# innate2adaptive/decombinator

Measured on AMD Instinct MI355X. Metric: Mreads/s decombined (150 bp human-beta), higher is better.
Workload: dtype u8

## Files before the change

### decombinator_amd/csrc/dcrx_kernels_v2.hip

```cpp
#include <hip/hip_runtime.h>
#include <hip/hip_ext.h>

#include <algorithm>
#include <cstddef>
#include <cstdio>
#include <cstdlib>
#include <vector>

#include "../../include/dcrx.h"
#include "dcrx_device.h"
#include "dcrx_launch.h"
#include "dcrx_dcr_device.h"
#include "dcrx_v2_device.h"
#include "dcrx_sink_device.h"

namespace dcrx {

bool first_use_on_device(bool (&seen)[64]);
void attributes_set_on_device(bool (&seen)[64]);

constexpr int DCRX_V2_BLOCK = 1024;
#ifdef DCRX_SCAN_STAMPS
__device__ uint32_t *g_scan_stamps;
#endif
// ... 287 lines not shown
  if (tid < DCRX_N_COUNTERS) lds_counts[tid] = 0;
  if (tid < V2_WK_WORDS) lds_work[tid] = 0;
  {
    const uint4 *src = reinterpret_cast<const uint4 *>(V0.trans);
    uint4 *dst = reinterpret_cast<uint4 *>(lds_trans);
    for (uint32_t i = tid; i < V0.trans_bytes / 16; i += blockDim.x) dst[i] = src[i];
  }
  const V2Tab tab{};
  uint32_t *lds_side = lds_work + V2_WK_WORDS;
  uint32_t *lds_bk = lds_side + (T0.lds_image_bytes - T0.dfa_bytes) / 4;
  uint32_t *ring = lds_bk + V0.bk_bytes / 4;
  const uint32_t ring_mask = 64u * ring_batches - 1u;
  constexpr uint32_t ES = (uint32_t)v2_ering_stride<NW>(), ering_mask = 64u * V2_ERING_BATCHES - 1u;
  uint32_t *ring2 = ring + (size_t)(ring_mask + 1u) * V2_RING_STRIDE;
  uint32_t *lds_dry = ring2 + (size_t)(ering_mask + 1u) * ES;
  if (FUSE >= 0) {
    {
      const uint4 *s1 = reinterpret_cast<const uint4 *>(T0.image + T0.dfa_bytes), *s2 = reinterpret_cast<const uint4 *>(V0.bk);
      uint4 *d1 = reinterpret_cast<uint4 *>(lds_side), *d2 = reinterpret_cast<uint4 *>(lds_bk);
      for (uint32_t i = tid; i < (T0.lds_image_bytes - T0.dfa_bytes) / 16; i += blockDim.x) d1[i] = s1[i];
      for (uint32_t i = tid; i < V0.bk_bytes / 16; i += blockDim.x) d2[i] = s2[i];
    }
    for (uint32_t i = tid; i <= ring_mask; i += blockDim.x) { ring[i * V2_RING_STRIDE + NW] = 0u; ring[i * V2_RING_STRIDE + NW + 1] = 0u; }
    if (FUSE_E) for (uint32_t i = tid; i <= ering_mask; i += blockDim.x) { ring2[i * ES + NW] = 0u; ring2[i * ES + NW + 1] = 0u; }
  }
  __syncthreads();
  const uint32_t nw = B.stride >> 2;
  const int lane = tid & 63;
  const unsigned long long lt_mask = (1ull << lane) - 1ull;
  const bool tagged = B.n_reads < (1ull << 30);

  const uint64_t blk_lo = (uint64_t)blockIdx.x * per_block;
  const uint64_t blk_hi = blk_lo + per_block < B.n_reads ? blk_lo + per_block : B.n_reads;
  uint32_t e_lo = 0u, e_hi = 0u;
  if (B.n_exc) {
    v2_exc_slice(B, blk_lo < blk_hi ? blk_lo : blk_hi, blk_hi, lds_work + V2_WK_EXC, tid);
    e_lo = lds_work[V2_WK_EXC]; e_hi = lds_work[V2_WK_EXC + 2];
    v2_exc_marks(B, e_lo, e_hi, true, tid);
    asm volatile("s_waitcnt vmcnt(0)" ::: "memory");
// ... 252 lines not shown
  }
  if (FUSE >= 0 && lane == 0) {
    asm volatile("s_waitcnt lgkmcnt(0)" ::: "memory");
    atomicAdd(&lds_work[V2_WK_SCANNED], 1u);
  }
  }
  if (FUSE_E && (wv >= n_scan_waves + tw || (DCRX_V2_HELP_DRAIN && scans))) {
   if constexpr (FUSE_E) {
    constexpr bool REV = FUSE == 1;
#if DCRX_V2_PRIO_TAIL
    __builtin_amdgcn_s_setprio(DCRX_V2_PRIO_TAIL);
#endif
    uint32_t kw_base[K_NCLASS];
#pragma unroll
    for (int c = 0; c < K_NCLASS; c++) kw_base[c] = T0.kw_base[c];
    const Rescue2Tabs rt = rescue2_tabs(T0, V0, reinterpret_cast<const uint8_t *>(lds_side), reinterpret_cast<const uint8_t *>(lds_bk), REV, kw_base);
    const Counters C{lds_counts}, Cdry{lds_dry};
    constexpr uint32_t nb_mask = V2_ERING_BATCHES - 1u, nb_shift = (uint32_t)__builtin_ctz(V2_ERING_BATCHES);
    constexpr uint32_t V2_RING_EXIT = 0xFFFFFFFFu;
    for (uint32_t spins = 0;;) {
      uint32_t c = 0, nvalid = 0;
      if (lane == 0) {
        c = __hip_atomic_load(&lds_work[V2_WK_CLAIM2], __ATOMIC_RELAXED, __HIP_MEMORY_SCOPE_WORKGROUP);
        const bool mine = __hip_atomic_load(&lds_work[V2_WK_GEN2 + (c & nb_mask)], __ATOMIC_RELAXED, __HIP_MEMORY_SCOPE_WORKGROUP) == (c >> nb_shift);
        const uint32_t f = __hip_atomic_load(&lds_work[V2_WK_FILLED2 + (c & nb_mask)], __ATOMIC_RELAXED, __HIP_MEMORY_SCOPE_WORKGROUP);
        if (!mine) nvalid = 0;
        else if (f == 64u) nvalid = 64u;
        else if (__hip_atomic_load(&lds_work[V2_WK_SCANNED], __ATOMIC_RELAXED, __HIP_MEMORY_SCOPE_WORKGROUP) == n_scan_waves) {
          const uint32_t h = __hip_atomic_load(&lds_work[V2_WK_HEAD2], __ATOMIC_RELAXED, __HIP_MEMORY_SCOPE_WORKGROUP);
          const uint32_t rem = h - 64u * c;
          nvalid = (int32_t)rem <= 0 ? V2_RING_EXIT : min(rem, 64u);
// ... 3 lines not shown
          if (!__hip_atomic_compare_exchange_strong(&lds_work[V2_WK_CLAIM2], &expect, c + 1u, __ATOMIC_RELAXED, __ATOMIC_RELAXED, __HIP_MEMORY_SCOPE_WORKGROUP)) nvalid = 0;
        }
      }
      c = (uint32_t)__builtin_amdgcn_readfirstlane((int)c);
      nvalid = (uint32_t)__builtin_amdgcn_readfirstlane((int)nvalid);
      if (nvalid == V2_RING_EXIT) break;
      if (!nvalid) {
        if (++spins > (1u << 24)) { if (lane == 0) atomicAdd(&counters[DCRX_C_DEVICE_ERRORS], 1ull); break; }
        __builtin_amdgcn_s_sleep(4);
        continue;
      }
      asm volatile("s_waitcnt lgkmcnt(0)" ::: "memory");
      uint32_t *sl = ring2 + ((64u * c + (uint32_t)lane) & ering_mask) * ES;
      int status = -2;
      uint32_t errs = 0, x0 = 0;
      uint32_t lg[NW];
#pragma unroll
      for (int k = 0; k < NW; k++) lg[k] = 0u;
      if ((uint32_t)lane < nvalid) {
        x0 = sl[NW + 2];
#pragma unroll
        for (int k = 0; k < NW; k++) lg[k] = sl[NW + 3 + k];
        const uint32_t dg = sl[2 * NW + 3];
        const uint32_t r = x0 & V2_R_MASK;
        const int n = UNIFORM_LEN ? (int)B.read_len : (int)B.lens[r];
        const LdsWords lw{dcrx_ldsaddr_of(sl)};
        auto on_ok = [&](dcrx_record_t rec, const uint32_t) {
          rec.frame = (uint8_t)(o ? 0 : 1);
          DCRX_STORE_FINISH(records + r, rec);
        };
        status = rescue2_fast_to<REV, NW, V2_SHAPE_ONE>(rt, lw, lg, n, cfg, on_ok, errs, *Tmem, C, Cdry, dg);
        if (status > 0) {
          dcrx_record_t rec;
          rec.v = rec.j = rec.v_start = rec.j_end = rec.ins_start = rec.ins_len = 0; rec.vdel = rec.jdel = 0;
          rec.status = (uint8_t)status; rec.frame = (uint8_t)(o ? 0 : 1);
          DCRX_STORE_FINISH(records + r, rec);
        } else if (status < 0) errs = 0;
      }
      v2_tally_rescue(lds_counts, lane, status, errs, o == 0);
      if (__builtin_expect(status == RESCUE2_SLOW, 0)) {
        uint32_t ww[NW];
#pragma unroll
        for (int k = 0; k < NW; k++) ww[k] = sl[k];
        if (!v2_left_push<NW>(Q.left, queue_count, x0, lg, ww)) v2_hand_over(B, queue, gqueue, qcap, queue_count, tagged, x0 & V2_R_MASK, false);
      }
      asm volatile("s_waitcnt lgkmcnt(0)" ::: "memory");
      if (lane == 0) {
        __hip_atomic_store(&lds_work[V2_WK_FILLED2 + (c & nb_mask)], 0u, __ATOMIC_RELAXED, __HIP_MEMORY_SCOPE_WORKGROUP);
        asm volatile("s_waitcnt lgkmcnt(0)" ::: "memory");
        atomicAdd(&lds_work[V2_WK_GEN2 + (c & nb_mask)], 1u);
      }
      spins = 0;
    }
   }
  }
  if (FUSE >= 0 && (DCRX_V2_HELP_DRAIN || (wv >= n_scan_waves && wv < n_scan_waves + tw))) {
   if constexpr (FUSE >= 0) {
    constexpr bool REV = FUSE == 1;
// ... 129 lines not shown
    x0e = (int)lo;
    while (lo < B.n_exc && B.exc_read[lo] == r) lo++;
    x1e = (int)lo;
    ExcLayout xl;
    if (x1e - x0e > V2_MAX_EXC && !exc_layout(B.exc_pos, B.exc_chr, x0e, x1e, xl)) {
      v2_hand_over(B, queue, gqueue, qcap, queue_count, tagged, r, true); return;
    }
  }
  if (!finish2_words<UNIFORM_LEN, NW, ORI>(T, V, B, cfg, (uint64_t)r, w, ev, (x0 & V2_R_JMULTI) != 0u, x0e, x1e, C, records))
    v2_hand_over(B, queue, gqueue, qcap, queue_count, tagged, r, exc);
}

constexpr int V2_LEFT_SLOTS = 15;
struct V2FinishLds {
  uint32_t *counts, *side, *bk, *strip, *dry, *left;
};
template <int NW, int BLOCK>
__device__ __forceinline__ V2FinishLds v2_finish_layout(const DevTables &T0, const V2Ori &V, uint32_t *smem, const int tid) {
  V2FinishLds L;
  L.counts = smem;
  L.side = smem + DCRX_N_COUNTERS;
  L.bk = L.side + (T0.lds_image_bytes - T0.dfa_bytes) / 4;
  L.strip = L.bk + V.bk_bytes / 4 + (uint32_t)tid * lds_words_stride<NW>();
  L.dry = L.bk + V.bk_bytes / 4 + (uint32_t)BLOCK * lds_words_stride<NW>();
  L.left = L.dry + DCRX_N_COUNTERS + (uint32_t)(tid >> 6) * (1 + V2_LEFT_SLOTS);
  return L;
}
template <int NW, int BLOCK>
__device__ __forceinline__ V2FinishLds v2_finish_stage(const DevTables &T0, const V2Ori &V, uint32_t *smem, const int tid) {
  const V2FinishLds L = v2_finish_layout<NW, BLOCK>(T0, V, smem, tid);
  if (tid < DCRX_N_COUNTERS) L.counts[tid] = 0;
  stage_lds<BLOCK>(T0.image + T0.dfa_bytes, L.side, (T0.lds_image_bytes - T0.dfa_bytes) / 16, 0, 0, tid);
  stage_lds<BLOCK>(V.bk, L.bk, V.bk_bytes / 16, 0, 0, tid);
  L.strip[NW] = 0u; L.strip[NW + 1] = 0u;
  if ((tid & 63) == 0) L.left[0] = 0u;
  return L;
}
template <int NW>
static uint32_t v2_finish_block_lds(const DevTables &T, int o, int block) {
  return DCRX_N_COUNTERS * 4 + (T.lds_image_bytes - T.dfa_bytes) + T.v2[o].bk_bytes + (uint32_t)block * lds_words_stride<NW>() * 4 + DCRX_N_COUNTERS * 4 +
         (uint32_t)(block / 64) * (1 + V2_LEFT_SLOTS) * 4;
}

__device__ __forceinline__ void v2_note_left(uint32_t *left, const uint32_t slot, const BatchDev &B, uint32_t *__restrict__ queue, uint32_t *__restrict__ gqueue,
                                             const uint32_t qcap, uint32_t *__restrict__ queue_count, const uint32_t r, const bool exc) {
  const uint32_t at = atomicAdd(&left[0], 1u);
  if (at < (uint32_t)V2_LEFT_SLOTS) left[1 + at] = slot;
  else v2_hand_over(B, queue, gqueue, qcap, queue_count, B.n_reads < (1ull << 30), r, exc);
}
template <int NW>
struct V2EntryWords { uint32_t lg[NW], w[NW]; };
template <bool UNIFORM_LEN, int NW, int ORI>
__device__ __forceinline__ void v2_tail_jobs(const Tail2Tabs &tt, const V2FinishLds &L, const BatchDev &B, const CfgDev &cfg, dcrx_record_t *__restrict__ records,
                                             const V2Lists &Q, const uint32_t n_regions, const uint32_t split, uint32_t *__restrict__ queue,
                                             uint32_t *__restrict__ gqueue, const uint32_t qcap, uint32_t *__restrict__ queue_count,
                                             const DevTables *__restrict__ Tmem, const uint32_t gwave, const uint32_t n_gwaves, const int tid, const V2SinkCall &S) {
// ... 104 lines not shown
      uint32_t x[2 + 2 * NW];
      const bool more = next_first < en;
      uint32_t after_raw = 0;
      uint32_t nf = next_first;
      if constexpr (AHEAD) {
#pragma unroll
        for (int k = 0; k < 2 + 2 * NW; k++) x[k] = x1[k];
        nf = v2_landed(x, next_first);
      }
      if (more && lane == 0) after_raw = __hip_atomic_fetch_add(tickets + V2_L_COUNTS * region + V2_L_TICKETS, which == V2_L_E ? 1u : 0x10000u, __ATOMIC_RELAXED, __HIP_MEMORY_SCOPE_AGENT);
      if constexpr (AHEAD) {
        v2_get_rows<2 + 2 * NW>(l.rows, l.cap, nf + lane, nf + lane < en, x1);
      } else {
        v2_get_rows<2 + 2 * NW>(l.rows, l.cap, first + lane, first + lane < en, x);
      }
      uint32_t lg[NW], w[NW];
#pragma unroll
      for (int k = 0; k < NW; k++) { lg[k] = x[1 + k]; w[k] = x[1 + NW + k]; }
      int status = -2;
      uint32_t errs = 0;
      uint64_t tup = 0;
      const uint32_t r = x[0] & V2_R_MASK;
      if (first + lane < en) {
        status = RESCUE2_SLOW;
        if (!(x[0] & V2_R_EXC)) {
          const int n = UNIFORM_LEN ? (int)B.read_len : (int)B.lens[r];
#pragma unroll
          for (int k = 0; k < NW; k++) strip[k] = w[k];
          auto on_ok = [&](dcrx_record_t rec, const uint32_t e) {
            rec.frame = (uint8_t)(o ? 0 : 1);
            DCRX_STORE_FINISH(records + r, rec);
            if (S.dev) tup = sink_tuple_lean(rec, S.wpack, (e & 8u) != 0u && 2 * rt.split[1] != (int)rt.t.L[1]);
          };
          if (which == V2_L_E) status = rescue2_fast_to<ORI == 1, NW, V2_SHAPE_ONE>(rt, lw, lg, n, cfg, on_ok, errs, *Tmem, C, Cdry, x[1 + 2 * NW]);
          else status = rescue2_fast_to<ORI == 1, NW, V2_SHAPE_BOTH>(rt, lw, lg, n, cfg, on_ok, errs, *Tmem, C, Cdry, x[1 + 2 * NW]);
          if (status > 0) {
            dcrx_record_t rec;
            rec.v = rec.j = rec.v_start = rec.j_end = rec.ins_start = rec.ins_len = 0; rec.vdel = rec.jdel = 0;
            rec.status = (uint8_t)status; rec.frame = (uint8_t)(o ? 0 : 1);
            DCRX_STORE_FINISH(records + r, rec);
          } else if (status < 0) errs = 0;
        }
      }
      v2_tally_rescue(lds_counts, lane, status, errs, o == 0);
      if (S.dev) sink_put(S, region, which == V2_L_E ? S.e_off : S.c_off, first + (uint32_t)lane, first + lane < en, status == DCRX_S_OK, r, tup, lane, nullptr);
      if (__builtin_expect(status == RESCUE2_SLOW, 0)) v2_note_left(s_left, first + (uint32_t)lane, B, queue, gqueue, qcap, queue_count, r, (x[0] & V2_R_EXC) != 0u);
      first = next_first;
      if (more) {
        const uint32_t t = (uint32_t)__builtin_amdgcn_readfirstlane((int)after_raw);
        next_first = 64u * (split + (which == V2_L_E ? (t & 0xFFFFu) : (t >> 16)));
// ... 68 lines not shown
  A.S.items = v2_global(A.S.items); A.S.hits = v2_global(A.S.hits);
  return A;
}
template <bool UNIFORM_LEN, int NW, int ORI, bool SINK>
DCRX_V2_ROLE void v2_rescue_role(const uint32_t vblock_, const uint32_t ka_lo, const uint32_t ka_hi) {
  extern __shared__ __align__(64) uint32_t smem[];
  V2FinishLocals A = v2_finish_args(ka_lo, ka_hi);
  if constexpr (!SINK) A.S.dev = nullptr;
  const uint32_t vblock = (uint32_t)__builtin_amdgcn_readfirstlane((int)vblock_);
  const int tid = threadIdx.x;
  const V2Ori V = A.T0.v2[ORI];
  const V2FinishLds L = v2_finish_layout<NW, DCRX_V2_FBLOCK>(A.T0, V, smem, tid);
  uint32_t kw_base[K_NCLASS];
#pragma unroll
  for (int c = 0; c < K_NCLASS; c++) kw_base[c] = A.T0.kw_base[c];
  const Rescue2Tabs rt = rescue2_tabs(A.T0, V, reinterpret_cast<const uint8_t *>(L.side), reinterpret_cast<const uint8_t *>(L.bk), ORI == 1, kw_base);
  constexpr uint32_t WPB = DCRX_V2_FBLOCK / 64;
  v2_rescue_jobs<UNIFORM_LEN, NW, ORI>(rt, L, A.B, A.cfg, A.records, A.Q, A.n_regions, A.R.rsplit, A.queue, A.gqueue, A.qcap, A.queue_count, A.Tmem,
                                       vblock * WPB + (uint32_t)(tid >> 6), A.R.rgrid * WPB, tid, A.S, A.tickets);
}
template <bool UNIFORM_LEN, int NW, int ORI, bool SINK>
DCRX_V2_ROLE void v2_tail_role(const uint32_t vblock_, const uint32_t ka_lo, const uint32_t ka_hi) {
  extern __shared__ __align__(64) uint32_t smem[];
  V2FinishLocals A = v2_finish_args(ka_lo, ka_hi);
  if constexpr (!SINK) A.S.dev = nullptr;
  const uint32_t vblock = (uint32_t)__builtin_amdgcn_readfirstlane((int)vblock_);
  const int tid = threadIdx.x;
  const V2Ori V = A.T0.v2[ORI];
  const V2FinishLds L = v2_finish_layout<NW, DCRX_V2_FBLOCK>(A.T0, V, smem, tid);
  const Tail2Tabs tt = tail2_tabs(A.T0, V, reinterpret_cast<const uint8_t *>(L.side), reinterpret_cast<const uint8_t *>(L.bk), ORI == 1);
  constexpr uint32_t WPB = DCRX_V2_FBLOCK / 64;
// ... 81 lines not shown
  bool work = true;
  if (b < R.xgrid) {
    role = 0;
    const uint32_t g = b / R.bsplit;
    work = g < A.n_regions && R.width * (DCRX_V2_FBLOCK / 64) * (b % R.bsplit) < A.Q.counts[V2_L_COUNTS * g + V2_L_X];
  } else {
    b -= R.xgrid;
    const uint32_t paired = 2u * min(R.rgrid, R.tgrid);
    if (b < paired) { role = (b & 1u) ? 2 : 1; b >>= 1; }
    else { b -= paired; role = R.rgrid > R.tgrid ? 1 : 2; b += min(R.rgrid, R.tgrid); }
  }
  const V2Ori V = A.T0.v2[ORI];
  V2FinishLds L = v2_finish_layout<NW, DCRX_V2_FBLOCK>(A.T0, V, smem, tid);
  const bool staged = work || blockIdx.x == 0;
  if (staged) {
    L = v2_finish_stage<NW, DCRX_V2_FBLOCK>(A.T0, V, smem, tid);
    __syncthreads();
    if (role == 1) v2_rescue_role<UNIFORM_LEN, NW, ORI, SINK>(b, (uint32_t)ka, (uint32_t)(ka >> 32));
    else if (TAIL_ROLE && role == 2) v2_tail_role<UNIFORM_LEN, NW, ORI, SINK>(b, (uint32_t)ka, (uint32_t)(ka >> 32));
    else v2_general_role<UNIFORM_LEN, NW, ORI, SINK>(blockIdx.x == 0 ? 3u : 1u, b, (uint32_t)ka, (uint32_t)(ka >> 32));
  }
  __syncthreads();
  if (blockIdx.x != 0 && tid == 0) atomicAdd(A.queue_count + V2_QC_DONE, 1u);
  __syncthreads();
  if (staged && tid < DCRX_N_COUNTERS && L.counts[tid]) atomicAdd(&A.counters[tid], (unsigned long long)L.counts[tid]);
}

template <bool UNIFORM_LEN, int NW, int ORI>
__global__ __launch_bounds__(DCRX_V2_FBLOCK, DCRX_V2_RWAVES) void left2_kernel(const V2FinishArgs A) {
  extern __shared__ __align__(64) uint32_t smem[];
  const int tid = threadIdx.x;
  if (A.queue_count[V2_QC_LEFT] == 0u) return;
  if (tid == 0) A.queue_count[V2_QC_DONE] = A.R.xgrid + A.R.rgrid + A.R.tgrid;
  __syncthreads();
  const uint64_t ka = (uint64_t)__builtin_amdgcn_kernarg_segment_ptr();
  const V2Ori V = A.T0.v2[ORI];
  const V2FinishLds L = v2_finish_stage<NW, DCRX_V2_FBLOCK>(A.T0, V, smem, tid);
  __syncthreads();
  v2_general_role<UNIFORM_LEN, NW, ORI, false>(2u, 0u, (uint32_t)ka, (uint32_t)(ka >> 32));
  __syncthreads();
  if (tid < DCRX_N_COUNTERS && L.counts[tid]) atomicAdd(&A.counters[tid], (unsigned long long)L.counts[tid]);
}

template <bool UNIFORM_LEN, int NW, int ORI>
__global__ __launch_bounds__(DCRX_V2_TBLOCK, DCRX_V2_TWAVES) void tail2_kernel(
    DevTables T0, BatchDev B, CfgDev cfg, dcrx_record_t *__restrict__ records, unsigned long long *__restrict__ counters,
    V2Lists Q, uint32_t n_regions, uint32_t split, uint32_t *__restrict__ queue, uint32_t *__restrict__ gqueue, uint32_t qcap,
    uint32_t *__restrict__ queue_count, const DevTables *__restrict__ Tmem) {
  extern __shared__ __align__(64) uint32_t smem[];
  const int tid = threadIdx.x;
  const V2Ori V = T0.v2[ORI];
  const V2FinishLds L = v2_finish_stage<NW, DCRX_V2_TBLOCK>(T0, V, smem, tid);
  const Tail2Tabs tt = tail2_tabs(T0, V, reinterpret_cast<const uint8_t *>(L.side), reinterpret_cast<const uint8_t *>(L.bk), ORI == 1);
  __syncthreads();
  v2_tail_jobs<UNIFORM_LEN, NW, ORI>(tt, L, B, cfg, records, Q, n_regions, split, queue, gqueue, qcap, queue_count, Tmem,
                                     blockIdx.x * (DCRX_V2_TBLOCK / 64) + (uint32_t)(tid >> 6), gridDim.x * (DCRX_V2_TBLOCK / 64), tid, V2SinkCall{});
  __syncthreads();
  if (tid < DCRX_N_COUNTERS && L.counts[tid]) atomicAdd(&counters[tid], (unsigned long long)L.counts[tid]);
}

template <bool UNIFORM_LEN, int NW, int ORI>
__global__ __launch_bounds__(DCRX_V2_FBLOCK, DCRX_V2_RWAVES) void rescue2_kernel(
    DevTables T0, BatchDev B, CfgDev cfg, dcrx_record_t *__restrict__ records, unsigned long long *__restrict__ counters,
    V2Lists Q, uint32_t n_regions, uint32_t split, uint32_t *__restrict__ queue, uint32_t *__restrict__ gqueue, uint32_t qcap,
    uint32_t *__restrict__ queue_count, const DevTables *__restrict__ Tmem) {
  extern __shared__ __align__(64) uint32_t smem[];
  const int tid = threadIdx.x;
  const V2Ori V = T0.v2[ORI];
  const V2FinishLds L = v2_finish_stage<NW, DCRX_V2_FBLOCK>(T0, V, smem, tid);
  uint32_t kw_base[K_NCLASS];
#pragma unroll
  for (int c = 0; c < K_NCLASS; c++) kw_base[c] = T0.kw_base[c];
  const Rescue2Tabs rt = rescue2_tabs(T0, V, reinterpret_cast<const uint8_t *>(L.side), reinterpret_cast<const uint8_t *>(L.bk), ORI == 1, kw_base);
  __syncthreads();
  v2_rescue_jobs<UNIFORM_LEN, NW, ORI>(rt, L, B, cfg, records, Q, n_regions, split, queue, gqueue, qcap, queue_count, Tmem,
                                       blockIdx.x * (DCRX_V2_FBLOCK / 64) + (uint32_t)(tid >> 6), gridDim.x * (DCRX_V2_FBLOCK / 64), tid, V2SinkCall{}, Q.counts);
  __syncthreads();
  if (tid < DCRX_N_COUNTERS && L.counts[tid]) atomicAdd(&counters[tid], (unsigned long long)L.counts[tid]);
}

template <bool UNIFORM_LEN, int NW, int ORI>
__global__ __launch_bounds__(DCRX_V2_FBLOCK, 4) void events2_kernel(
    DevTables T0, BatchDev B, CfgDev cfg, dcrx_record_t *__restrict__ records, unsigned long long *__restrict__ counters,
    V2Lists Q, int which, uint32_t group, uint32_t width, uint32_t bsplit, uint32_t ext, uint32_t n_regions, uint32_t *__restrict__ queue, uint32_t *__restrict__ gqueue, uint32_t qcap,
    uint32_t *__restrict__ queue_count) {
  extern __shared__ __align__(64) uint32_t smem[];
  V2Ori V = T0.v2[ORI];
  const uint32_t lcap = v2_list<NW>(Q, which, 0).cap;
// ... 242 lines not shown
        if (ready) {
          float ms[2] = {0.f, 0.f};
          for (int a = 0; a < 2 * NP && ok; a++) { float t = 0.f; ok = hipEventElapsedTime(&t, eslot->ev_e[a][0], eslot->ev_e[a][1]) == hipSuccess; ms[a < NP ? 0 : 1] += t; }
          eslot->us_e[0] = 1e3f * ms[0] / NP; eslot->us_e[1] = 1e3f * ms[1] / NP;
          eslot->fuse_e = (ok && ms[1] > 0.f && ms[1] < 0.985f * ms[0]) ? 1 : 0;
          want = eslot->fuse_e == 1;
          static const bool say = dcrx_debug_env("DCRX_DEBUG_TUNE") != nullptr;
          if (say) fprintf(stderr, "dcrx tune: scan + finishing launch of %llu reads, frame %d: %.1f us with list E a role, %.1f inside the scan -> %s\n",
                           (unsigned long long)B.n_reads, o, eslot->us_e[0], eslot->us_e[1], eslot->fuse_e ? "inside the scan" : "a role");
        }
      }
      (void)hipGetLastError();
    }
    if (ring_batches && want && !retry && !(cfg.flags & ~(DCRX_F_V2_SHAPE(3)))) {
      const uint32_t fixed = v2_scan_lds_bytes(T, o) + (T.lds_image_bytes - T.dfa_bytes) + T.v2[o].bk_bytes + 64u * V2_ERING_BATCHES * (uint32_t)v2_ering_stride<NW>() * 4u +
                             DCRX_N_COUNTERS * 4u;
      for (uint32_t nb = ring_batches; nb >= 8u; nb >>= 1)
        if (fixed + nb * 64u * V2_RING_STRIDE * 4u <= 160u * 1024u) { ring_batches_e = nb; scan_lds_e = fixed + nb * 64u * V2_RING_STRIDE * 4u; break; }
      if (!ring_batches_e && eslot && fuse_e_env < 0) eslot->fuse_e = 0;
      if (ring_batches_e) {
        fuse_e = true;
        ks_e = o ? scan2_kernel<UNIFORM, NW, RPL, NARROW, PREFETCH, 1, false, true> : scan2_kernel<UNIFORM, NW, RPL, NARROW, PREFETCH, 0, false, true>;
      }
    }
  }
  if (P.tune && ring_batches) P.tune[o].last_form = 3u;
  const uint32_t scan_lds = v2_scan_lds_bytes(T, o) + (ring_batches ? (T.lds_image_bytes - T.dfa_bytes) + T.v2[o].bk_bytes + ring_batches * 64u * V2_RING_STRIDE * 4u : 0u);
  auto ke = o ? events2_kernel<UNIFORM, NW, 1> : events2_kernel<UNIFORM, NW, 0>;
  auto kt = o ? tail2_kernel<UNIFORM, NW, 1> : tail2_kernel<UNIFORM, NW, 0>;
  auto kr = o ? rescue2_kernel<UNIFORM, NW, 1> : rescue2_kernel<UNIFORM, NW, 0>;
  auto kf = o ? finish2_kernel<UNIFORM, NW, 1> : finish2_kernel<UNIFORM, NW, 0>;
// ... 357 lines not shown
```

### decombinator_amd/csrc/dcrx_v2_device.h

```cpp
#pragma once

#include "dcrx_dcr_device.h"

namespace dcrx {

#ifndef DCRX_HOST_EMUL
DCRX_DEV uint32_t dcrx_alignbit(uint32_t hi, uint32_t lo, uint32_t sh) { return __builtin_amdgcn_alignbit(hi, lo, sh); }
typedef __attribute__((address_space(3))) uint16_t dcrx_lds_u16;
struct V2Tab {};
DCRX_DEV uint32_t v2_entry(const V2Tab &, uint32_t byte_off) {
  return *reinterpret_cast<const dcrx_lds_u16 *>(static_cast<uintptr_t>(byte_off));
}
#else
inline uint32_t dcrx_alignbit(uint32_t hi, uint32_t lo, uint32_t sh) { return (uint32_t)((((uint64_t)hi << 32) | lo) >> (sh & 31)); }
struct V2Tab { const uint16_t *base; };
inline uint32_t v2_entry(const V2Tab &tab, uint32_t byte_off) { return tab.base[byte_off >> 1]; }
#endif

#ifndef DCRX_HOST_EMUL
typedef uint32_t dcrx_ldsaddr;
template <typename T>
DCRX_DEV T dcrx_lds_at(dcrx_ldsaddr a, uint32_t i) {
  return reinterpret_cast<const __attribute__((address_space(3))) T *>(static_cast<uintptr_t>(a))[i];
}
// ... 818 lines not shown
  else if (status == DCRX_S_J_WALK_FAIL) C.add(DCRX_C_VJ_ASSIGNMENT_FAILED);
  else if (status == DCRX_S_F_TOOLONG) C.add(DCRX_C_DCRFILTER_TOOLONG_INTERTAG);
  else if (status == DCRX_S_F_IMPOSS_DEL) C.add(DCRX_C_DCRFILTER_IMPOSS_DELETION);
  else if (status == DCRX_S_F_OVERLAP) C.add(DCRX_C_DCRFILTER_TAG_OVERLAP);
}

struct Rescue2Tabs {
  Tail2Tabs t;
  uint32_t h_mask[2][2];
  dcrx_ldsaddr h_kw[2][2], h_pk[2][2];
  dcrx_ldsaddr kw_begin, kw_tags;
  dcrx_ldsaddr tag_pk[2];
  uint32_t kw_base[2][2];
  uint32_t Lh[2][2];
  int32_t split[2];
};

DCRX_DEV Rescue2Tabs rescue2_tabs(const DevTables &T0, const V2Ori &V0, const uint8_t *side, const uint8_t *bk, const bool rev,
                                  const uint32_t (&kw_base)[K_NCLASS]) {
  Rescue2Tabs r;
  r.t = tail2_tabs(T0, V0, side, bk, rev);
  auto at_side = [&](const void *p) { return dcrx_ldsaddr_of(side + ((reinterpret_cast<const uint8_t *>(p) - T0.image) - T0.dfa_bytes)); };
  for (int g = 0; g < 2; g++) {
    for (int h = 0; h < 2; h++) {
      const int cls = g == 0 ? (h == 0 ? K_VH1 : K_VH2) : (h == 0 ? K_JH1 : K_JH2);
      r.h_mask[g][h] = V0.bk_mask[cls];
      r.h_kw[g][h] = dcrx_ldsaddr_of(bk + V0.bk_kw_off[cls]);
      r.h_pk[g][h] = dcrx_ldsaddr_of(bk + V0.bk_pk_off[cls]);
      r.kw_base[g][h] = kw_base[cls];
      r.Lh[g][h] = T0.kw_len[cls];
    }
    r.tag_pk[g] = at_side(rev ? T0.g[g].tag_pk_rc : T0.g[g].tag_pk_fwd);
    r.split[g] = T0.g[g].split;
  }
  r.kw_begin = at_side(T0.kw_begin);
  r.kw_tags = at_side(T0.kw_tags);
  return r;
}

constexpr int RESCUE2_SLOW = -1;
#if defined(DCRX_HOST_EMUL) && defined(DCRX_R2_PROFILE)
void r2_prof(int what, int a);
#define R2P(what, a) r2_prof(what, a)
#else
#define R2P(what, a) ((void)0)
#endif
#ifdef DCRX_R2_REASONS
extern unsigned long long g_r2_reasons[32];
#define R2S(k) (g_r2_reasons[k]++, RESCUE2_SLOW)
#else
#define R2S(k) RESCUE2_SLOW
#endif

template <int G>
struct GeneOf {
  const Rescue2Tabs &rt;
  bool j;
  DCRX_DEV uint32_t h_mask(int h) const { return G >= 0 ? rt.h_mask[G < 0 ? 0 : G][h] : (j ? rt.h_mask[1][h] : rt.h_mask[0][h]); }
  DCRX_DEV dcrx_ldsaddr h_kw(int h) const { return G >= 0 ? rt.h_kw[G < 0 ? 0 : G][h] : (j ? rt.h_kw[1][h] : rt.h_kw[0][h]); }
  DCRX_DEV dcrx_ldsaddr h_pk(int h) const { return G >= 0 ? rt.h_pk[G < 0 ? 0 : G][h] : (j ? rt.h_pk[1][h] : rt.h_pk[0][h]); }
  DCRX_DEV uint32_t kw_base(int h) const { return G >= 0 ? rt.kw_base[G < 0 ? 0 : G][h] : (j ? rt.kw_base[1][h] : rt.kw_base[0][h]); }
  DCRX_DEV int Lh(int h) const { return (int)(G >= 0 ? rt.Lh[G < 0 ? 0 : G][h] : (j ? rt.Lh[1][h] : rt.Lh[0][h])); }
  DCRX_DEV dcrx_ldsaddr tag_pk() const { return G >= 0 ? rt.tag_pk[G < 0 ? 0 : G] : (j ? rt.tag_pk[1] : rt.tag_pk[0]); }
  DCRX_DEV int Lt() const { return (int)(G >= 0 ? rt.t.L[G < 0 ? 0 : G] : (j ? rt.t.L[1] : rt.t.L[0])); }
  DCRX_DEV int split() const { return G >= 0 ? rt.split[G < 0 ? 0 : G] : (j ? rt.split[1] : rt.split[0]); }
  DCRX_DEV uint32_t fbit() const { return G >= 0 ? (G == 0 ? V2_F_VH : V2_F_JH) : (j ? V2_F_JH : V2_F_VH); }
};

template <bool REV, class WS, int G>
DCRX_DEV int rescue2_candidates(const GeneOf<G> &g, const WS &w, const int n, const int half, const uint32_t gk,
                                const int p, int &k_out, int &q_out) {
  const Rescue2Tabs &rt = g.rt;
  const int L = g.Lt();
  const int q = half == 1 ? p : p - g.split();
  if (q + L < 0) return R2S(1);
  if (q < 0 || q + L > n) return 0;
  const int b = REV ? n - q - L : q;
  const int ws = min(b, n - 32);
  const uint64_t mask = (1ull << (2 * L)) - 1ull;
  const uint64_t val = (w.stored64(ws) >> (2 * (b - ws))) & mask;
  const uint32_t x0 = dcrx_lds_at<uint32_t>(rt.kw_begin, gk), x1 = dcrx_lds_at<uint32_t>(rt.kw_begin, gk + 1);
// ... 3 lines not shown
    R2P(5, half);
    const int k = (int)dcrx_lds_at<uint32_t>(rt.kw_tags, x);
    const uint64_t y = mismatch_slots(val, dcrx_lds_at<uint64_t>(tpk, (uint32_t)k)) & mask;
    if (dcrx_popc64(y) <= 1) { found = 1; k_out = k; q_out = q; }
  }
  return found;
}

template <int NW>
DCRX_DEV uint32_t log_word(const uint32_t (&lg)[NW], const int kk) {
  uint32_t l = 0;
#pragma unroll
  for (int k = 0; k < NW; k++) l = (kk == k) ? lg[k] : l;
  return l;
}

template <bool REV, int NW, class WS, int G>
DCRX_DEV int rescue2_half(const GeneOf<G> &g, const WS &w, const uint32_t (&lg)[NW], const int n,
                          int &k_out, int &q_out, int &p_out, int &half_out) {
  const int L1 = g.Lh(0), L2 = g.Lh(1);
  const uint64_t m1 = (1ull << (2 * L1)) - 1ull, m2 = (1ull << (2 * L2)) - 1ull;
  const uint32_t mask8 = g.fbit() * 0x11111111u;
  uint32_t nz = 0;
#pragma unroll
  for (int kk = 0; kk < NW; kk++) nz |= (lg[kk] & mask8) ? (1u << kk) : 0u;
  uint64_t h2lo = 0, h2hi = 0;
  int h2n = 0;
  bool any1 = false;
  int res = 0;
  R2P(1, G);
  while (nz && res == 0) {
    R2P(2, 0);
    const int kk = REV ? 31 - dcrx_clz32(nz) : dcrx_ctz32(nz);
    nz &= ~(1u << kk);
    uint32_t m = log_word<NW>(lg, kk) & mask8;
    while (m && res == 0) {
      R2P(3, 0);
      const int bit = REV ? 31 - dcrx_clz32(m) : dcrx_ctz32(m);
      m &= ~(1u << bit);
      const int pair = 8 * kk + (bit >> 2);
      const int f1 = 2 * pair + 1;
      const int xs = f1 >= 31 ? f1 - 31 : 0;
      const uint64_t X = w.stored64(xs);
      for (int y = 0; y < 2 && res == 0; y++) {
        const int f = REV ? f1 - y : f1 - 1 + y;
        if (f >= n) continue;
        R2P(4, y);
        const int s1 = f - L1 + 1, s2 = f - L2 + 1;
        const LookupQ q[2] = {{g.h_mask(0), g.h_kw(0), g.h_pk(0), (X >> v2_sh(s1 - xs)) & m1, s1 >= 0},
                              {g.h_mask(1), g.h_kw(1), g.h_pk(1), (X >> v2_sh(s2 - xs)) & m2, s2 >= 0}};
// ... 28 lines not shown
    res = rescue2_candidates<REV, WS, G>(g, w, n, 2, g.kw_base(1) + (uint32_t)kw2, p, k_out, q_out);
    p_out = p;
  }
  return res;
}

enum { V2_SHAPE_ANY = -1, V2_SHAPE_ONE = 0, V2_SHAPE_BOTH = 1 };
DCRX_DEV int shape2(const uint32_t vf_n, const uint32_t jf_n, const uint32_t any) {
  return (vf_n == 0u && jf_n == 0u && (any & V2_F_JH)) ? V2_SHAPE_BOTH : V2_SHAPE_ONE;
}

constexpr uint32_t RESCUE2_NO_DIGEST = 0xFFFFFFFFu;
DCRX_DEV uint32_t rescue2_digest_pack(const Digest2 &d) {
  return min(d.vf_n, 3u) | (min(d.jf_n, 3u) << 2) | ((d.any & 0xFu) << 4) | ((d.vf_pair & 0xFFu) << 8) | ((d.jf_pair & 0xFFu) << 16);
}
template <bool REV, int NW, int SHAPE, class WS, class OnOk>
DCRX_DEV int rescue2_fast_to(const Rescue2Tabs &rt, const WS &w, const uint32_t (&lg)[NW], const int n, const CfgDev &cfg,
                             OnOk &&on_ok, uint32_t &errs, const DevTables &T, const Counters &C, const Counters &Cdry,
                             const uint32_t dg = RESCUE2_NO_DIGEST) {
  const Tail2Tabs &tt = rt.t;
  const int Lv = (int)tt.L[0], Lj = (int)tt.L[1];
  errs = 0;
  if (n < 32 || Lv > 31 || Lj > 31) return R2S(2);
  uint32_t vfn = 0, jfn = 0, any = 0, vf1 = 0xFFFFFFFFu, jf1 = 0xFFFFFFFFu;
  if (dg != RESCUE2_NO_DIGEST) {
    vfn = dg & 3u; jfn = (dg >> 2) & 3u; any = (dg >> 4) & 0xFu;
    vf1 = ((dg >> 8) & 0xFFu) << 2; jf1 = ((dg >> 16) & 0xFFu) << 2;
  } else {
#pragma unroll
    for (int kk = 0; kk < NW; kk++) {
      const uint32_t l = lg[kk];
      any |= l;
      if (SHAPE != V2_SHAPE_BOTH) {
        const uint32_t tv = l & 0x11111111u, tj = l & 0x22222222u;
        const uint32_t kb = (uint32_t)kk << 5;
        vfn += (uint32_t)dcrx_popc64(tv);
        vf1 = min(vf1, (tv ? (uint32_t)dcrx_ctz32(tv) : 0xFFFFFFFFu) | kb);
        jfn += (uint32_t)dcrx_popc64(tj);
        jf1 = min(jf1, (tj ? (uint32_t)dcrx_ctz32(tj) : 0xFFFFFFFFu) | kb);
      }
    }
    any |= any >> 16; any |= any >> 8; any |= any >> 4; any &= 0xFu;
  }
  if ((n & 1) && log_nibble<NW>(lg, n >> 1)) return R2S(3);
  if (vfn > 1 || (vfn == 0 && !(any & V2_F_VH))) return R2S(4);
  const bool vfull = vfn == 1;
  const bool jsweep = jfn == 0 && (any & V2_F_JH) != 0u;
  if (SHAPE == V2_SHAPE_ONE && vfull != jsweep) return R2S(4);
  if (SHAPE == V2_SHAPE_BOTH && (vfull || !jsweep)) return R2S(4);
  const uint64_t mv = (1ull << (2 * Lv)) - 1ull, mj = (1ull << (2 * Lj)) - 1ull;

  int ftag = -1, fs = 0;
  const bool jfull = !vfull && jfn == 1;
  if (SHAPE != V2_SHAPE_BOTH && (vfull || jfull)) {
    const int Lf = vfull ? Lv : Lj;
    const uint64_t mf = vfull ? mv : mj;
    const int pair = (int)((vfull ? vf1 : jf1) >> 2);
    const int sa = 2 * pair - Lf + 1;
    const int ws = min(max(sa, 0), n - 32);
// ... 87 lines not shown
  int lo, hi;
  pyslice(n, end_v + 1, start_j, lo, hi);
  dcrx_record_t rec;
  rec.v = (uint16_t)v; rec.j = (uint16_t)j;
  rec.v_start = (uint16_t)vp; rec.j_end = (uint16_t)jend;
  rec.ins_start = (uint16_t)lo; rec.ins_len = (uint16_t)(hi - lo);
  rec.vdel = (uint8_t)kv; rec.jdel = (uint8_t)kj;
  rec.status = (uint8_t)DCRX_S_OK; rec.frame = 0;
  on_ok(rec, errs);
  return DCRX_S_OK;
}
template <bool REV, int NW, int SHAPE, class WS>
DCRX_DEV int rescue2_fast(const Rescue2Tabs &rt, const WS &w, const uint32_t (&lg)[NW], const int n, const CfgDev &cfg,
                          dcrx_record_t &rec, uint32_t &errs, const DevTables &T, const Counters &C, const Counters &Cdry,
                          const uint32_t dg = RESCUE2_NO_DIGEST) {
  return rescue2_fast_to<REV, NW, SHAPE>(rt, w, lg, n, cfg, [&](const dcrx_record_t &r, const uint32_t) {
    rec.v = r.v; rec.j = r.j; rec.v_start = r.v_start; rec.j_end = r.j_end; rec.ins_start = r.ins_start; rec.ins_len = r.ins_len;
    rec.vdel = r.vdel; rec.jdel = r.jdel; }, errs, T, C, Cdry, dg);
}

DCRX_DEV void rescue2_count(const Counters &C, const int status, const uint32_t errs, const bool forward) {
  C.add(DCRX_C_READ_COUNT);
  if (errs & 1u) C.add(DCRX_C_VERR1);
  if (errs & 2u) C.add(DCRX_C_VERR2);
  if (errs & 4u) C.add(DCRX_C_JERR1);
  if (errs & 8u) C.add(DCRX_C_JERR2);
  switch (status) {
    case DCRX_S_OK: C.add(DCRX_C_VJ_COUNT); if (forward) C.add(DCRX_C_FRAME_FORWARD); break;
    case DCRX_S_V_HALF1_EXHAUSTED: C.add(DCRX_C_FOUNDV1NOTV2); break;
    case DCRX_S_V_HALF2_EXHAUSTED: C.add(DCRX_C_FOUNDV2NOTV1); break;
    case DCRX_S_V_NONE: C.add(DCRX_C_NO_VTAGS_FOUND); break;
// ... 14 lines not shown
```

Baseline: 33600.

## Stage gene table records in LDS and read rescue log words from LDS

Per-gene rescue table fields (masks, keyword addresses, lengths, split) are written once per block into a small LDS record. When the gene is chosen at runtime they are read from that record instead of being selected from registers. In the fused E-ring consumer, the log words are no longer copied into a register array; they are read from the ring slot in LDS through a new LdsLog accessor. The aim is to cut VGPR pressure in the rescue path, at the cost of extra LDS reads and a little more LDS per block.

```diff
diff --git a/decombinator_amd/csrc/dcrx_kernels_v2.hip b/decombinator_amd/csrc/dcrx_kernels_v2.hip
--- a/decombinator_amd/csrc/dcrx_kernels_v2.hip
+++ b/decombinator_amd/csrc/dcrx_kernels_v2.hip
@@ -325,6 +325,7 @@
   constexpr uint32_t ES = (uint32_t)v2_ering_stride<NW>(), ering_mask = 64u * V2_ERING_BATCHES - 1u;
   uint32_t *ring2 = ring + (size_t)(ring_mask + 1u) * V2_RING_STRIDE;
   uint32_t *lds_dry = ring2 + (size_t)(ering_mask + 1u) * ES;
+  uint32_t *lds_gene = lds_dry + DCRX_N_COUNTERS;
   if (FUSE >= 0) {
     {
       const uint4 *s1 = reinterpret_cast<const uint4 *>(T0.image + T0.dfa_bytes), *s2 = reinterpret_cast<const uint4 *>(V0.bk);
@@ -334,6 +335,12 @@
     }
     for (uint32_t i = tid; i <= ring_mask; i += blockDim.x) { ring[i * V2_RING_STRIDE + NW] = 0u; ring[i * V2_RING_STRIDE + NW + 1] = 0u; }
     if (FUSE_E) for (uint32_t i = tid; i <= ering_mask; i += blockDim.x) { ring2[i * ES + NW] = 0u; ring2[i * ES + NW + 1] = 0u; }
+    if (FUSE_E && tid == 0) {
+      uint32_t kw_base[K_NCLASS];
+#pragma unroll
+      for (int c = 0; c < K_NCLASS; c++) kw_base[c] = T0.kw_base[c];
+      rescue2_stage_genes(rescue2_tabs(T0, V0, reinterpret_cast<const uint8_t *>(lds_side), reinterpret_cast<const uint8_t *>(lds_bk), FUSE == 1, kw_base), lds_gene);
+    }
   }
   __syncthreads();
   const uint32_t nw = B.stride >> 2;
@@ -616,7 +623,7 @@
     uint32_t kw_base[K_NCLASS];
 #pragma unroll
     for (int c = 0; c < K_NCLASS; c++) kw_base[c] = T0.kw_base[c];
-    const Rescue2Tabs rt = rescue2_tabs(T0, V0, reinterpret_cast<const uint8_t *>(lds_side), reinterpret_cast<const uint8_t *>(lds_bk), REV, kw_base);
+    const Rescue2Tabs rt = rescue2_tabs(T0, V0, reinterpret_cast<const uint8_t *>(lds_side), reinterpret_cast<const uint8_t *>(lds_bk), REV, kw_base, lds_gene);
     const Counters C{lds_counts}, Cdry{lds_dry};
     constexpr uint32_t nb_mask = V2_ERING_BATCHES - 1u, nb_shift = (uint32_t)__builtin_ctz(V2_ERING_BATCHES);
     constexpr uint32_t V2_RING_EXIT = 0xFFFFFFFFu;
@@ -650,22 +657,18 @@
       uint32_t *sl = ring2 + ((64u * c + (uint32_t)lane) & ering_mask) * ES;
       int status = -2;
       uint32_t errs = 0, x0 = 0;
-      uint32_t lg[NW];
-#pragma unroll
-      for (int k = 0; k < NW; k++) lg[k] = 0u;
       if ((uint32_t)lane < nvalid) {
         x0 = sl[NW + 2];
-#pragma unroll
-        for (int k = 0; k < NW; k++) lg[k] = sl[NW + 3 + k];
         const uint32_t dg = sl[2 * NW + 3];
         const uint32_t r = x0 & V2_R_MASK;
         const int n = UNIFORM_LEN ? (int)B.read_len : (int)B.lens[r];
         const LdsWords lw{dcrx_ldsaddr_of(sl)};
+        const LdsLog ll{dcrx_ldsaddr_of(sl + NW + 3)};
         auto on_ok = [&](dcrx_record_t rec, const uint32_t) {
           rec.frame = (uint8_t)(o ? 0 : 1);
           DCRX_STORE_FINISH(records + r, rec);
         };
-        status = rescue2_fast_to<REV, NW, V2_SHAPE_ONE>(rt, lw, lg, n, cfg, on_ok, errs, *Tmem, C, Cdry, dg);
+        status = rescue2_fast_to<REV, NW, V2_SHAPE_ONE>(rt, lw, ll, n, cfg, on_ok, errs, *Tmem, C, Cdry, dg);
         if (status > 0) {
           dcrx_record_t rec;
           rec.v = rec.j = rec.v_start = rec.j_end = rec.ins_start = rec.ins_len = 0; rec.vdel = rec.jdel = 0;
@@ -675,9 +678,9 @@
       }
       v2_tally_rescue(lds_counts, lane, status, errs, o == 0);
       if (__builtin_expect(status == RESCUE2_SLOW, 0)) {
-        uint32_t ww[NW];
-#pragma unroll
-        for (int k = 0; k < NW; k++) ww[k] = sl[k];
+        uint32_t lg[NW], ww[NW];
+#pragma unroll
+        for (int k = 0; k < NW; k++) { lg[k] = sl[NW + 3 + k]; ww[k] = sl[k]; }
         if (!v2_left_push<NW>(Q.left, queue_count, x0, lg, ww)) v2_hand_over(B, queue, gqueue, qcap, queue_count, tagged, x0 & V2_R_MASK, false);
       }
       asm volatile("s_waitcnt lgkmcnt(0)" ::: "memory");
@@ -837,6 +840,7 @@
 constexpr int V2_LEFT_SLOTS = 15;
 struct V2FinishLds {
   uint32_t *counts, *side, *bk, *strip, *dry, *left;
+  uint32_t *gene;
 };
 template <int NW, int BLOCK>
 __device__ __forceinline__ V2FinishLds v2_finish_layout(const DevTables &T0, const V2Ori &V, uint32_t *smem, const int tid) {
@@ -847,22 +851,29 @@
   L.strip = L.bk + V.bk_bytes / 4 + (uint32_t)tid * lds_words_stride<NW>();
   L.dry = L.bk + V.bk_bytes / 4 + (uint32_t)BLOCK * lds_words_stride<NW>();
   L.left = L.dry + DCRX_N_COUNTERS + (uint32_t)(tid >> 6) * (1 + V2_LEFT_SLOTS);
+  L.gene = L.dry + DCRX_N_COUNTERS + (uint32_t)(BLOCK / 64) * (1 + V2_LEFT_SLOTS);
   return L;
 }
 template <int NW, int BLOCK>
-__device__ __forceinline__ V2FinishLds v2_finish_stage(const DevTables &T0, const V2Ori &V, uint32_t *smem, const int tid) {
+__device__ __forceinline__ V2FinishLds v2_finish_stage(const DevTables &T0, const V2Ori &V, uint32_t *smem, const int tid, const bool rev) {
   const V2FinishLds L = v2_finish_layout<NW, BLOCK>(T0, V, smem, tid);
   if (tid < DCRX_N_COUNTERS) L.counts[tid] = 0;
   stage_lds<BLOCK>(T0.image + T0.dfa_bytes, L.side, (T0.lds_image_bytes - T0.dfa_bytes) / 16, 0, 0, tid);
   stage_lds<BLOCK>(V.bk, L.bk, V.bk_bytes / 16, 0, 0, tid);
   L.strip[NW] = 0u; L.strip[NW + 1] = 0u;
   if ((tid & 63) == 0) L.left[0] = 0u;
+  if (tid == 0) {
+    uint32_t kw_base[K_NCLASS];
+#pragma unroll
+    for (int c = 0; c < K_NCLASS; c++) kw_base[c] = T0.kw_base[c];
+    rescue2_stage_genes(rescue2_tabs(T0, V, reinterpret_cast<const uint8_t *>(L.side), reinterpret_cast<const uint8_t *>(L.bk), rev, kw_base), L.gene);
+  }
   return L;
 }
 template <int NW>
 static uint32_t v2_finish_block_lds(const DevTables &T, int o, int block) {
   return DCRX_N_COUNTERS * 4 + (T.lds_image_bytes - T.dfa_bytes) + T.v2[o].bk_bytes + (uint32_t)block * lds_words_stride<NW>() * 4 + DCRX_N_COUNTERS * 4 +
-         (uint32_t)(block / 64) * (1 + V2_LEFT_SLOTS) * 4;
+         (uint32_t)(block / 64) * (1 + V2_LEFT_SLOTS) * 4 + 2 * R2G_WORDS * 4;
 }
 
 __device__ __forceinline__ void v2_note_left(uint32_t *left, const uint32_t slot, const BatchDev &B, uint32_t *__restrict__ queue, uint32_t *__restrict__ gqueue,
@@ -997,9 +1008,6 @@
       } else {
         v2_get_rows<2 + 2 * NW>(l.rows, l.cap, first + lane, first + lane < en, x);
       }
-      uint32_t lg[NW], w[NW];
-#pragma unroll
-      for (int k = 0; k < NW; k++) { lg[k] = x[1 + k]; w[k] = x[1 + NW + k]; }
       int status = -2;
       uint32_t errs = 0;
       uint64_t tup = 0;
@@ -1008,15 +1016,17 @@
         status = RESCUE2_SLOW;
         if (!(x[0] & V2_R_EXC)) {
           const int n = UNIFORM_LEN ? (int)B.read_len : (int)B.lens[r];
-#pragma unroll
-          for (int k = 0; k < NW; k++) strip[k] = w[k];
+          uint32_t lg[NW];
+#pragma unroll
+          for (int k = 0; k < NW; k++) { lg[k] = x[1 + k]; strip[k] = x[1 + NW + k]; }
+          const RegLog<NW> rl{lg};
           auto on_ok = [&](dcrx_record_t rec, const uint32_t e) {
             rec.frame = (uint8_t)(o ? 0 : 1);
             DCRX_STORE_FINISH(records + r, rec);
             if (S.dev) tup = sink_tuple_lean(rec, S.wpack, (e & 8u) != 0u && 2 * rt.split[1] != (int)rt.t.L[1]);
           };
-          if (which == V2_L_E) status = rescue2_fast_to<ORI == 1, NW, V2_SHAPE_ONE>(rt, lw, lg, n, cfg, on_ok, errs, *Tmem, C, Cdry, x[1 + 2 * NW]);
-          else status = rescue2_fast_to<ORI == 1, NW, V2_SHAPE_BOTH>(rt, lw, lg, n, cfg, on_ok, errs, *Tmem, C, Cdry, x[1 + 2 * NW]);
+          if (which == V2_L_E) status = rescue2_fast_to<ORI == 1, NW, V2_SHAPE_ONE>(rt, lw, rl, n, cfg, on_ok, errs, *Tmem, C, Cdry, x[1 + 2 * NW]);
+          else status = rescue2_fast_to<ORI == 1, NW, V2_SHAPE_BOTH>(rt, lw, rl, n, cfg, on_ok, errs, *Tmem, C, Cdry, x[1 + 2 * NW]);
           if (status > 0) {
             dcrx_record_t rec;
             rec.v = rec.j = rec.v_start = rec.j_end = rec.ins_start = rec.ins_len = 0; rec.vdel = rec.jdel = 0;
@@ -1115,7 +1125,7 @@
   uint32_t kw_base[K_NCLASS];
 #pragma unroll
   for (int c = 0; c < K_NCLASS; c++) kw_base[c] = A.T0.kw_base[c];
-  const Rescue2Tabs rt = rescue2_tabs(A.T0, V, reinterpret_cast<const uint8_t *>(L.side), reinterpret_cast<const uint8_t *>(L.bk), ORI == 1, kw_base);
+  const Rescue2Tabs rt = rescue2_tabs(A.T0, V, reinterpret_cast<const uint8_t *>(L.side), reinterpret_cast<const uint8_t *>(L.bk), ORI == 1, kw_base, L.gene);
   constexpr uint32_t WPB = DCRX_V2_FBLOCK / 64;
   v2_rescue_jobs<UNIFORM_LEN, NW, ORI>(rt, L, A.B, A.cfg, A.records, A.Q, A.n_regions, A.R.rsplit, A.queue, A.gqueue, A.qcap, A.queue_count, A.Tmem,
                                        vblock * WPB + (uint32_t)(tid >> 6), A.R.rgrid * WPB, tid, A.S, A.tickets);
@@ -1227,7 +1237,7 @@
   V2FinishLds L = v2_finish_layout<NW, DCRX_V2_FBLOCK>(A.T0, V, smem, tid);
   const bool staged = work || blockIdx.x == 0;
   if (staged) {
-    L = v2_finish_stage<NW, DCRX_V2_FBLOCK>(A.T0, V, smem, tid);
+    L = v2_finish_stage<NW, DCRX_V2_FBLOCK>(A.T0, V, smem, tid, ORI == 1);
     __syncthreads();
     if (role == 1) v2_rescue_role<UNIFORM_LEN, NW, ORI, SINK>(b, (uint32_t)ka, (uint32_t)(ka >> 32));
     else if (TAIL_ROLE && role == 2) v2_tail_role<UNIFORM_LEN, NW, ORI, SINK>(b, (uint32_t)ka, (uint32_t)(ka >> 32));
@@ -1248,7 +1258,7 @@
   __syncthreads();
   const uint64_t ka = (uint64_t)__builtin_amdgcn_kernarg_segment_ptr();
   const V2Ori V = A.T0.v2[ORI];
-  const V2FinishLds L = v2_finish_stage<NW, DCRX_V2_FBLOCK>(A.T0, V, smem, tid);
+  const V2FinishLds L = v2_finish_stage<NW, DCRX_V2_FBLOCK>(A.T0, V, smem, tid, ORI == 1);
   __syncthreads();
   v2_general_role<UNIFORM_LEN, NW, ORI, false>(2u, 0u, (uint32_t)ka, (uint32_t)(ka >> 32));
   __syncthreads();
@@ -1263,7 +1273,7 @@
   extern __shared__ __align__(64) uint32_t smem[];
   const int tid = threadIdx.x;
   const V2Ori V = T0.v2[ORI];
-  const V2FinishLds L = v2_finish_stage<NW, DCRX_V2_TBLOCK>(T0, V, smem, tid);
+  const V2FinishLds L = v2_finish_stage<NW, DCRX_V2_TBLOCK>(T0, V, smem, tid, ORI == 1);
   const Tail2Tabs tt = tail2_tabs(T0, V, reinterpret_cast<const uint8_t *>(L.side), reinterpret_cast<const uint8_t *>(L.bk), ORI == 1);
   __syncthreads();
   v2_tail_jobs<UNIFORM_LEN, NW, ORI>(tt, L, B, cfg, records, Q, n_regions, split, queue, gqueue, qcap, queue_count, Tmem,
@@ -1280,11 +1290,11 @@
   extern __shared__ __align__(64) uint32_t smem[];
   const int tid = threadIdx.x;
   const V2Ori V = T0.v2[ORI];
-  const V2FinishLds L = v2_finish_stage<NW, DCRX_V2_FBLOCK>(T0, V, smem, tid);
+  const V2FinishLds L = v2_finish_stage<NW, DCRX_V2_FBLOCK>(T0, V, smem, tid, ORI == 1);
   uint32_t kw_base[K_NCLASS];
 #pragma unroll
   for (int c = 0; c < K_NCLASS; c++) kw_base[c] = T0.kw_base[c];
-  const Rescue2Tabs rt = rescue2_tabs(T0, V, reinterpret_cast<const uint8_t *>(L.side), reinterpret_cast<const uint8_t *>(L.bk), ORI == 1, kw_base);
+  const Rescue2Tabs rt = rescue2_tabs(T0, V, reinterpret_cast<const uint8_t *>(L.side), reinterpret_cast<const uint8_t *>(L.bk), ORI == 1, kw_base, L.gene);
   __syncthreads();
   v2_rescue_jobs<UNIFORM_LEN, NW, ORI>(rt, L, B, cfg, records, Q, n_regions, split, queue, gqueue, qcap, queue_count, Tmem,
                                        blockIdx.x * (DCRX_V2_FBLOCK / 64) + (uint32_t)(tid >> 6), gridDim.x * (DCRX_V2_FBLOCK / 64), tid, V2SinkCall{}, Q.counts);
@@ -1557,7 +1567,7 @@
     }
     if (ring_batches && want && !retry && !(cfg.flags & ~(DCRX_F_V2_SHAPE(3)))) {
       const uint32_t fixed = v2_scan_lds_bytes(T, o) + (T.lds_image_bytes - T.dfa_bytes) + T.v2[o].bk_bytes + 64u * V2_ERING_BATCHES * (uint32_t)v2_ering_stride<NW>() * 4u +
-                             DCRX_N_COUNTERS * 4u;
+                             DCRX_N_COUNTERS * 4u + 2u * R2G_WORDS * 4u;
       for (uint32_t nb = ring_batches; nb >= 8u; nb >>= 1)
         if (fixed + nb * 64u * V2_RING_STRIDE * 4u <= 160u * 1024u) { ring_batches_e = nb; scan_lds_e = fixed + nb * 64u * V2_RING_STRIDE * 4u; break; }
       if (!ring_batches_e && eslot && fuse_e_env < 0) eslot->fuse_e = 0;
diff --git a/decombinator_amd/csrc/dcrx_v2_device.h b/decombinator_amd/csrc/dcrx_v2_device.h
--- a/decombinator_amd/csrc/dcrx_v2_device.h
+++ b/decombinator_amd/csrc/dcrx_v2_device.h
@@ -856,10 +856,12 @@
   uint32_t kw_base[2][2];
   uint32_t Lh[2][2];
   int32_t split[2];
+  dcrx_ldsaddr gene_rec;
 };
+enum { R2G_HMASK = 0, R2G_HKW = 2, R2G_HPK = 4, R2G_KWBASE = 6, R2G_LH = 8, R2G_TAGPK = 10, R2G_LT = 11, R2G_SPLIT = 12, R2G_FBIT = 13, R2G_WORDS = 16 };
 
 DCRX_DEV Rescue2Tabs rescue2_tabs(const DevTables &T0, const V2Ori &V0, const uint8_t *side, const uint8_t *bk, const bool rev,
-                                  const uint32_t (&kw_base)[K_NCLASS]) {
+                                  const uint32_t (&kw_base)[K_NCLASS], const void *gene_rec = nullptr) {
   Rescue2Tabs r;
   r.t = tail2_tabs(T0, V0, side, bk, rev);
   auto at_side = [&](const void *p) { return dcrx_ldsaddr_of(side + ((reinterpret_cast<const uint8_t *>(p) - T0.image) - T0.dfa_bytes)); };
@@ -877,8 +879,24 @@
   }
   r.kw_begin = at_side(T0.kw_begin);
   r.kw_tags = at_side(T0.kw_tags);
+  r.gene_rec = dcrx_ldsaddr_of(gene_rec);
   return r;
 }
+
+#ifndef DCRX_HOST_EMUL
+DCRX_DEV void rescue2_stage_genes(const Rescue2Tabs &rt, uint32_t *rec) {
+#pragma unroll
+  for (int g = 0; g < 2; g++) {
+    uint32_t *r = rec + g * R2G_WORDS;
+#pragma unroll
+    for (int h = 0; h < 2; h++) {
+      r[R2G_HMASK + h] = rt.h_mask[g][h]; r[R2G_HKW + h] = rt.h_kw[g][h]; r[R2G_HPK + h] = rt.h_pk[g][h];
+      r[R2G_KWBASE + h] = rt.kw_base[g][h]; r[R2G_LH + h] = rt.Lh[g][h];
+    }
+    r[R2G_TAGPK] = rt.tag_pk[g]; r[R2G_LT] = rt.t.L[g]; r[R2G_SPLIT] = (uint32_t)rt.split[g];
+  }
+}
+#endif
 
 constexpr int RESCUE2_SLOW = -1;
 #if defined(DCRX_HOST_EMUL) && defined(DCRX_R2_PROFILE)
@@ -898,6 +916,24 @@
 struct GeneOf {
   const Rescue2Tabs &rt;
   bool j;
+#ifndef DCRX_HOST_EMUL
+#define DCRX_R2G(EXPR, IDX) (G >= 0 ? (uint32_t)(EXPR) : rec(IDX))
+  DCRX_DEV uint32_t rec(const int i) const {
+    const dcrx_ldsaddr a = rt.gene_rec + (j ? (uint32_t)R2G_WORDS * 4u : 0u);
+    asm volatile("" ::: "memory");
+    return dcrx_lds_at<uint32_t>(a, (uint32_t)i);
+  }
+  DCRX_DEV uint32_t h_mask(int h) const { return DCRX_R2G(rt.h_mask[G < 0 ? 0 : G][h], R2G_HMASK + h); }
+  DCRX_DEV dcrx_ldsaddr h_kw(int h) const { return DCRX_R2G(rt.h_kw[G < 0 ? 0 : G][h], R2G_HKW + h); }
+  DCRX_DEV dcrx_ldsaddr h_pk(int h) const { return DCRX_R2G(rt.h_pk[G < 0 ? 0 : G][h], R2G_HPK + h); }
+  DCRX_DEV uint32_t kw_base(int h) const { return DCRX_R2G(rt.kw_base[G < 0 ? 0 : G][h], R2G_KWBASE + h); }
+  DCRX_DEV int Lh(int h) const { return (int)DCRX_R2G(rt.Lh[G < 0 ? 0 : G][h], R2G_LH + h); }
+  DCRX_DEV dcrx_ldsaddr tag_pk() const { return DCRX_R2G(rt.tag_pk[G < 0 ? 0 : G], R2G_TAGPK); }
+  DCRX_DEV int Lt() const { return (int)DCRX_R2G(rt.t.L[G < 0 ? 0 : G], R2G_LT); }
+  DCRX_DEV int split() const { return (int)DCRX_R2G((uint32_t)rt.split[G < 0 ? 0 : G], R2G_SPLIT); }
+  DCRX_DEV uint32_t fbit() const { return G >= 0 ? (G == 0 ? V2_F_VH : V2_F_JH) : (j ? V2_F_JH : V2_F_VH); }
+#undef DCRX_R2G
+#else
   DCRX_DEV uint32_t h_mask(int h) const { return G >= 0 ? rt.h_mask[G < 0 ? 0 : G][h] : (j ? rt.h_mask[1][h] : rt.h_mask[0][h]); }
   DCRX_DEV dcrx_ldsaddr h_kw(int h) const { return G >= 0 ? rt.h_kw[G < 0 ? 0 : G][h] : (j ? rt.h_kw[1][h] : rt.h_kw[0][h]); }
   DCRX_DEV dcrx_ldsaddr h_pk(int h) const { return G >= 0 ? rt.h_pk[G < 0 ? 0 : G][h] : (j ? rt.h_pk[1][h] : rt.h_pk[0][h]); }
@@ -907,6 +943,7 @@
   DCRX_DEV int Lt() const { return (int)(G >= 0 ? rt.t.L[G < 0 ? 0 : G] : (j ? rt.t.L[1] : rt.t.L[0])); }
   DCRX_DEV int split() const { return G >= 0 ? rt.split[G < 0 ? 0 : G] : (j ? rt.split[1] : rt.split[0]); }
   DCRX_DEV uint32_t fbit() const { return G >= 0 ? (G == 0 ? V2_F_VH : V2_F_JH) : (j ? V2_F_JH : V2_F_VH); }
+#endif
 };
 
 template <bool REV, class WS, int G>
@@ -940,16 +977,27 @@
   for (int k = 0; k < NW; k++) l = (kk == k) ? lg[k] : l;
   return l;
 }
-
-template <bool REV, int NW, class WS, int G>
-DCRX_DEV int rescue2_half(const GeneOf<G> &g, const WS &w, const uint32_t (&lg)[NW], const int n,
+template <int NW>
+struct RegLog {
+  const uint32_t (&lg)[NW];
+  DCRX_DEV uint32_t word(const int kk) const { return log_word<NW>(lg, kk); }
+};
+struct LdsLog {
+  dcrx_ldsaddr base;
+  DCRX_DEV uint32_t word(const int kk) const { return dcrx_lds_at<uint32_t>(base, (uint32_t)kk); }
+};
+template <class LG>
+DCRX_DEV uint32_t log_nibble_of(const LG &lg, const int pair) { return (lg.word(pair >> 3) >> (4 * (pair & 7))) & 0xFu; }
+
+template <bool REV, int NW, class WS, int G, class LG>
+DCRX_DEV int rescue2_half(const GeneOf<G> &g, const WS &w, const LG &lg, const int n,
                           int &k_out, int &q_out, int &p_out, int &half_out) {
   const int L1 = g.Lh(0), L2 = g.Lh(1);
   const uint64_t m1 = (1ull << (2 * L1)) - 1ull, m2 = (1ull << (2 * L2)) - 1ull;
   const uint32_t mask8 = g.fbit() * 0x11111111u;
   uint32_t nz = 0;
 #pragma unroll
-  for (int kk = 0; kk < NW; kk++) nz |= (lg[kk] & mask8) ? (1u << kk) : 0u;
+  for (int kk = 0; kk < NW; kk++) nz |= (lg.word(kk) & mask8) ? (1u << kk) : 0u;
   uint64_t h2lo = 0, h2hi = 0;
   int h2n = 0;
   bool any1 = false;
@@ -959,7 +1007,7 @@
     R2P(2, 0);
     const int kk = REV ? 31 - dcrx_clz32(nz) : dcrx_ctz32(nz);
     nz &= ~(1u << kk);
-    uint32_t m = log_word<NW>(lg, kk) & mask8;
+    uint32_t m = lg.word(kk) & mask8;
     while (m && res == 0) {
       R2P(3, 0);
       const int bit = REV ? 31 - dcrx_clz32(m) : dcrx_ctz32(m);
@@ -1018,8 +1066,8 @@
 DCRX_DEV uint32_t rescue2_digest_pack(const Digest2 &d) {
   return min(d.vf_n, 3u) | (min(d.jf_n, 3u) << 2) | ((d.any & 0xFu) << 4) | ((d.vf_pair & 0xFFu) << 8) | ((d.jf_pair & 0xFFu) << 16);
 }
-template <bool REV, int NW, int SHAPE, class WS, class OnOk>
-DCRX_DEV int rescue2_fast_to(const Rescue2Tabs &rt, const WS &w, const uint32_t (&lg)[NW], const int n, const CfgDev &cfg,
+template <bool REV, int NW, int SHAPE, class WS, class LG, class OnOk>
+DCRX_DEV int rescue2_fast_to(const Rescue2Tabs &rt, const WS &w, const LG &lg, const int n, const CfgDev &cfg,
                              OnOk &&on_ok, uint32_t &errs, const DevTables &T, const Counters &C, const Counters &Cdry,
                              const uint32_t dg = RESCUE2_NO_DIGEST) {
   const Tail2Tabs &tt = rt.t;
@@ -1033,7 +1081,7 @@
   } else {
 #pragma unroll
     for (int kk = 0; kk < NW; kk++) {
-      const uint32_t l = lg[kk];
+      const uint32_t l = lg.word(kk);
       any |= l;
       if (SHAPE != V2_SHAPE_BOTH) {
         const uint32_t tv = l & 0x11111111u, tj = l & 0x22222222u;
@@ -1046,7 +1094,7 @@
     }
     any |= any >> 16; any |= any >> 8; any |= any >> 4; any &= 0xFu;
   }
-  if ((n & 1) && log_nibble<NW>(lg, n >> 1)) return R2S(3);
+  if ((n & 1) && log_nibble_of(lg, n >> 1)) return R2S(3);
   if (vfn > 1 || (vfn == 0 && !(any & V2_F_VH))) return R2S(4);
   const bool vfull = vfn == 1;
   const bool jsweep = jfn == 0 && (any & V2_F_JH) != 0u;
@@ -1164,7 +1212,7 @@
 DCRX_DEV int rescue2_fast(const Rescue2Tabs &rt, const WS &w, const uint32_t (&lg)[NW], const int n, const CfgDev &cfg,
                           dcrx_record_t &rec, uint32_t &errs, const DevTables &T, const Counters &C, const Counters &Cdry,
                           const uint32_t dg = RESCUE2_NO_DIGEST) {
-  return rescue2_fast_to<REV, NW, SHAPE>(rt, w, lg, n, cfg, [&](const dcrx_record_t &r, const uint32_t) {
+  return rescue2_fast_to<REV, NW, SHAPE>(rt, w, RegLog<NW>{lg}, n, cfg, [&](const dcrx_record_t &r, const uint32_t) {
     rec.v = r.v; rec.j = r.j; rec.v_start = r.v_start; rec.j_end = r.j_end; rec.ins_start = r.ins_start; rec.ins_len = r.ins_len;
     rec.vdel = r.vdel; rec.jdel = r.jdel; }, errs, T, C, Cdry, dg);
 }
```

New measurement: 33600. No clear change (-0.0%).
